# Lynne-Zheng-Linfang/HS-Pose

Hardware: AMD Instinct MI355X
Metric: point-clouds/sec (N=1028) HS-layer fwd+bwd (higher is better)
Workload: dtype f32; 1 GPU; HS stack (FaceRecon backbone -> feat) fwd+bwd, B=16/GPU N=1028 fp32, train-mode BN, random-init weights (BASELINE configs[1] shape); global_batch=16, points=1028, parallelism=dp1, hipgraph=True, split_graph=False, grad_exchange=none

## Files before the change

### hs_pose_amd/csrc/gemm_x3.hip

```cpp
#include "common.h"
#include <stdlib.h>
#include <type_traits>

namespace hsp {

using f32x16 = __attribute__((ext_vector_type(16))) float;
using bf16x8 = __attribute__((ext_vector_type(8))) __bf16;
using u32x4 = __attribute__((ext_vector_type(4))) unsigned;

struct X3Args {
    const float* A[2];
    const unsigned short* P[2];
    int lda[2], ldp[2], K[2];
    long long ps[2];
    float* C; int ldc;
    int M, N;
    const float* bias;
    const float* resid; int ldr;
    const float* cbias; int rpc;
    float alpha;
    int tiles_m, tiles_n, nsplit;
    float* ws;
    float* bn_shift;
    float* bn_part;
};

#define X3_BN 128
#define X3_BK 32

__device__ __forceinline__ void x3_split8(const float (&x)[8], u32x4& hi, u32x4& mid, u32x4& lo) {
    float r1[8], r2[8];
#pragma unroll
    for (int i = 0; i < 8; ++i) {
        const float h = __uint_as_float(__float_as_uint(x[i]) & 0xffff0000u);
        r1[i] = x[i] - h;
        const float m = __uint_as_float(__float_as_uint(r1[i]) & 0xffff0000u);
        r2[i] = r1[i] - m;
    }
#pragma unroll
    for (int i = 0; i < 4; ++i) {
        hi[i] = __builtin_amdgcn_perm(__float_as_uint(x[2 * i + 1]), __float_as_uint(x[2 * i]), 0x07060302u);
        mid[i] = __builtin_amdgcn_perm(__float_as_uint(r1[2 * i + 1]), __float_as_uint(r1[2 * i]), 0x07060302u);
        lo[i] = __builtin_amdgcn_perm(__float_as_uint(r2[2 * i + 1]), __float_as_uint(r2[2 * i]), 0x07060302u);
    }
}

template <int WM, bool TWO, int EPI, int PA = 0>
__global__ __launch_bounds__(256, 2) void gemm_x3_kernel(const X3Args g) {
    constexpr int BM = 64 * WM;
    constexpr int A_PLANE = BM * 64, B_PLANE = X3_BN * 64;
    constexpr int NAU = WM;
    extern __shared__ __attribute__((aligned(16))) char smem[];
    char* sA = smem;
    char* sB = smem + 3 * A_PLANE;

    const int tid = threadIdx.x, lane = tid & 63;
    const int wave = __builtin_amdgcn_readfirstlane(tid >> 6);
    const int li = lane & 31, lh = lane >> 5;
    const int wm0 = (wave >> 1) * 32 * WM, wn0 = (wave & 1) * 64;

    const int item = blockIdx.x;
    const int o = item / g.nsplit, ks = item - o * g.nsplit;
    const int tm = o / g.tiles_n, tn = o - tm * g.tiles_n;
    const int m0 = tm * BM, n0 = tn * X3_BN;
    const int T0 = (g.K[0] + X3_BK - 1) / X3_BK;
    const int T1 = TWO ? (g.K[1] + X3_BK - 1) / X3_BK : 0;
    const int TT = T0 + T1;
    const int per = (TT + g.nsplit - 1) / g.nsplit;
    const int t_begin = ks * per, t_end = min(TT, t_begin + per);

    f32x16 acc[WM][2];
#pragma unroll
    for (int a = 0; a < WM; ++a)
#pragma unroll
        for (int b = 0; b < 2; ++b)
#pragma unroll
            for (int r = 0; r < 16; ++r) acc[a][b][r] = 0.f;
    if constexpr (EPI == 2) {
        const __amdgpu_buffer_rsrc_t rsR = __builtin_amdgcn_make_buffer_rsrc(
            const_cast<float*>(g.resid), 0, (int)((size_t)g.M * g.ldr * 4), 0x00020000);
        const unsigned ldr4 = (unsigned)g.ldr * 4u;
#pragma unroll
        for (int y = 0; y < 2; ++y) {
            const int col = n0 + wn0 + 32 * y + li;
            const unsigned voff = col < g.N ? (unsigned)(m0 + wm0 + 4 * lh) * ldr4 + (unsigned)col * 4u : 0xfffffff0u;
#pragma unroll
            for (int x = 0; x < WM; ++x)
#pragma unroll
                for (int r = 0; r < 16; ++r)
                    acc[x][y][r] = __uint_as_float(
                        __builtin_amdgcn_raw_buffer_load_b32(rsR, voff, (unsigned)(32 * x + (r & 3) + 8 * (r >> 2)) * ldr4, 0));
        }
    }

    u32x4 bv[6];
    const __amdgpu_buffer_rsrc_t rsA0 = __builtin_amdgcn_make_buffer_rsrc(
        const_cast<float*>(g.A[0]), 0, (int)((((size_t)g.M - 1) * g.lda[0] + g.K[0]) * 4), 0x00020000);
    const __amdgpu_buffer_rsrc_t rsA1 = __builtin_amdgcn_make_buffer_rsrc(
        const_cast<float*>(TWO ? g.A[1] : g.A[0]), 0, (int)((((size_t)g.M - 1) * g.lda[TWO ? 1 : 0] + g.K[TWO ? 1 : 0]) * 4), 0x00020000);
    auto fetchA = [&](float (&dst)[NAU][8], int t) {
        const int src = (TWO && t >= T0) ? 1 : 0;
        const int kb = (src ? t - T0 : t) * X3_BK;
        const __amdgpu_buffer_rsrc_t ra = src ? rsA1 : rsA0;
        const unsigned lda = (unsigned)g.lda[src];
#pragma unroll
        for (int i = 0; i < NAU; ++i) {
            const int u = tid + 256 * i, row = u >> 2, c8 = u & 3;
            const int gr = m0 + row, k0 = kb + 8 * c8;
            const unsigned off = gr < g.M ? ((unsigned)gr * lda + (unsigned)k0) * 4u : 0xfffffff0u;
            const u32x4 v0 = __builtin_amdgcn_raw_buffer_load_b128(ra, off, 0, 0);
            const u32x4 v1 = __builtin_amdgcn_raw_buffer_load_b128(ra, off, 16, 0);
#pragma unroll
            for (int e = 0; e < 4; ++e) { dst[i][e] = __uint_as_float(v0[e]); dst[i][4 + e] = __uint_as_float(v1[e]); }
        }
    };
    auto fetchB = [&](int t) {
        const int src = (TWO && t >= T0) ? 1 : 0;
        const int kb = (src ? t - T0 : t) * X3_BK;
        const unsigned short* P = g.P[src];
        const int ldp = g.ldp[src];
        const long long ps = g.ps[src];
#pragma unroll
        for (int i = 0; i < 6; ++i) {
            const int q = tid + 256 * i, plane = q >> 9, w = q & 511, row = w >> 2, c = w & 3;
            bv[i] = *reinterpret_cast<const u32x4*>(P + plane * ps + (size_t)min(n0 + row, g.N - 1) * ldp + kb + 8 * c);
        }
    };
    auto stashA = [&](float (&srcv)[NAU][8], int t) {
        {
            const int src = (TWO && t >= T0) ? 1 : 0;
            const int kb = (src ? t - T0 : t) * X3_BK, K = g.K[src];
            if (kb + X3_BK > K) {
#pragma unroll
                for (int i = 0; i < NAU; ++i) {
                    const int k0 = kb + 8 * ((tid + 256 * i) & 3);
#pragma unroll
                    for (int e = 0; e < 8; ++e) srcv[i][e] = k0 + e < K ? srcv[i][e] : 0.f;
                }
            }
        }
#pragma unroll
        for (int i = 0; i < NAU; ++i) {
            const int u = tid + 256 * i, row = u >> 2, c8 = u & 3;
            u32x4 h, m, l;
            x3_split8(srcv[i], h, m, l);
            const int off = row * 64 + ((c8 ^ ((row >> 2) & 3)) << 4);
            *reinterpret_cast<u32x4*>(sA + off) = h;
            *reinterpret_cast<u32x4*>(sA + A_PLANE + off) = m;
            *reinterpret_cast<u32x4*>(sA + 2 * A_PLANE + off) = l;
        }
    };
    auto stashB = [&]() {
#pragma unroll
        for (int i = 0; i < 6; ++i) {
            const int q = tid + 256 * i, plane = q >> 9, w = q & 511, row = w >> 2, c = w & 3;
            *reinterpret_cast<u32x4*>(sB + plane * B_PLANE + row * 64 + ((c ^ ((row >> 2) & 3)) << 4)) = bv[i];
        }
    };
    auto mma = [&]() {
#pragma unroll
        for (int s = 0; s < 2; ++s) {
            u32x4 fa[WM][3], fb[2][3];
            const int c = 2 * s + lh;
#pragma unroll
            for (int x = 0; x < WM; ++x) {
                const int row = wm0 + 32 * x + li;
                const int off = row * 64 + ((c ^ ((row >> 2) & 3)) << 4);
#pragma unroll
                for (int p = 0; p < 3; ++p) fa[x][p] = *reinterpret_cast<const u32x4*>(sA + p * A_PLANE + off);
            }
#pragma unroll
            for (int y = 0; y < 2; ++y) {
                const int row = wn0 + 32 * y + li;
                const int off = row * 64 + ((c ^ ((row >> 2) & 3)) << 4);
#pragma unroll
                for (int p = 0; p < 3; ++p) fb[y][p] = *reinterpret_cast<const u32x4*>(sB + p * B_PLANE + off);
            }
            constexpr int SA[6] = {0, 2, 1, 0, 1, 0}, SB[6] = {2, 0, 1, 1, 0, 0};
#pragma unroll
            for (int q = 0; q < 6; ++q)
#pragma unroll
                for (int x = 0; x < WM; ++x)
#pragma unroll
                    for (int y = 0; y < 2; ++y)
                        acc[x][y] = __builtin_amdgcn_mfma_f32_32x32x16_bf16(__builtin_bit_cast(bf16x8, fa[x][SA[q]]),
                                                                            __builtin_bit_cast(bf16x8, fb[y][SB[q]]), acc[x][y], 0, 0, 0);
        }
    };
    {
        float av[NAU][8];
        if (t_begin < t_end) { fetchA(av, t_begin); fetchB(t_begin); }
        for (int t = t_begin; t < t_end; ++t) {
            __syncthreads();
            stashA(av, t);
            stashB();
            __syncthreads();
            if (t + 1 < t_end) { fetchA(av, t + 1); fetchB(t + 1); }
            mma();
        }
    }

    if (g.nsplit > 1) {
        float* wsp = g.ws + (size_t)ks * g.M * g.N;
#pragma unroll
        for (int y = 0; y < 2; ++y) {
            const int col = n0 + wn0 + 32 * y + li;
#pragma unroll
            for (int x = 0; x < WM; ++x)
#pragma unroll
                for (int r = 0; r < 16; ++r) {
                    const int row = m0 + wm0 + 32 * x + (r & 3) + 8 * (r >> 2) + 4 * lh;
                    if (row < g.M && col < g.N) wsp[(size_t)row * g.N + col] = acc[x][y][r];
                }
        }
        return;
    }
    constexpr bool HAS_BIAS = EPI & 1, HAS_RES = (EPI & 2) && EPI != 2, HAS_CB = EPI & 4, HAS_BN = EPI & 8;
    float bn1[2] = {0.f, 0.f}, bn2[2] = {0.f, 0.f};
    const int c0 = m0 / g.rpc, nb = (c0 + 1) * g.rpc;
    const bool two_clouds = g.rpc >= BM;
#pragma unroll
    for (int y = 0; y < 2; ++y) {
        const int col = n0 + wn0 + 32 * y + li;
        const bool cok = col < g.N;
        const int colc = min(col, g.N - 1);
        float bvv = 0.f, cb0 = 0.f, cb1 = 0.f, bsh = 0.f;
        if constexpr (HAS_BIAS) bvv = g.bias[colc];
        if constexpr (HAS_BN) {
            if constexpr (HAS_RES) bsh = g.resid[colc] + g.cbias[colc];
            else bsh = bvv;
            if (tm == 0 && wm0 == 0 && lh == 0 && cok) g.bn_shift[col] = bsh;
        }
        if constexpr (HAS_CB) {
            cb0 = g.cbias[(size_t)c0 * g.N + colc];
            cb1 = g.cbias[(size_t)min(c0 + 1, (g.M - 1) / g.rpc) * g.N + colc];
        }
#pragma unroll
        for (int x = 0; x < WM; ++x) {
#pragma unroll
            for (int r4 = 0; r4 < 16; r4 += 4) {
                float rv[4];
                if constexpr (HAS_RES) {
#pragma unroll
                    for (int q = 0; q < 4; ++q) {
                        const int row = min(m0 + wm0 + 32 * x + q + 8 * (r4 >> 2) + 4 * lh, g.M - 1);
                        rv[q] = g.resid[(size_t)row * g.ldr + colc];
                    }
                }
#pragma unroll
                for (int q = 0; q < 4; ++q) {
                    const int r = r4 + q;
                    const int row = m0 + wm0 + 32 * x + q + 8 * (r4 >> 2) + 4 * lh;
                    float v = g.alpha * acc[x][y][r] + bvv;
                    if constexpr (HAS_RES) v += rv[q];
                    if constexpr (HAS_CB) {
                        if (two_clouds) v += row >= nb ? cb1 : cb0;
                        else v += g.cbias[(size_t)(min(row, g.M - 1) / g.rpc) * g.N + colc];
                    }
                    if (row < g.M && cok) g.C[(size_t)row * g.ldc + col] = v;
                    if constexpr (HAS_BN) {
                        const float d = row < g.M ? v - bsh : 0.f;
                        bn1[y] += d;
                        bn2[y] += d * d;
                    }
                }
            }
        }
    }
    if constexpr (HAS_BN) {
        __syncthreads();
        float* red = reinterpret_cast<float*>(smem);
#pragma unroll
        for (int y = 0; y < 2; ++y) {
            const float a = bn1[y] + __shfl_xor(bn1[y], 32, 64), b = bn2[y] + __shfl_xor(bn2[y], 32, 64);
            if (lh == 0) {
                red[((wave >> 1) * 2 + 0) * 128 + wn0 + 32 * y + li] = a;
                red[((wave >> 1) * 2 + 1) * 128 + wn0 + 32 * y + li] = b;
            }
        }
        __syncthreads();
        if (tid < 128 && n0 + tid < g.N) {
            g.bn_part[((size_t)tm * 2 + 0) * g.N + n0 + tid] = red[0 * 128 + tid] + red[2 * 128 + tid];
            g.bn_part[((size_t)tm * 2 + 1) * g.N + n0 + tid] = red[1 * 128 + tid] + red[3 * 128 + tid];
        }
    }
}

template <int EPI>
__global__ __launch_bounds__(256, 2) void gemm_x3_panel_kernel(const X3Args g) {
    constexpr int KS = 8, K = 128, D = 2;
    constexpr int ROWB = K * 2, PLANE = 32 * ROWB, BUF = 3 * PLANE;
    constexpr int UPR = K / 8, NAU = (32 * UPR) / 256;
    extern __shared__ __attribute__((aligned(16))) char smem[];
    char* sA = smem;

    const int tid = threadIdx.x, lane = tid & 63;
    const int wave = __builtin_amdgcn_readfirstlane(tid >> 6);
    const int li = lane & 31, lh = lane >> 5;
    const int P = g.tiles_n, R = gridDim.x / P;
    const int xq = blockIdx.x / HSP_NUM_XCD, xcd = blockIdx.x % HSP_NUM_XCD;
    const int panel = xq % P, slot = (xq / P) * HSP_NUM_XCD + xcd;
    const int col = panel * 128 + 32 * wave + li;
    const int ntiles = g.tiles_m;

    const __amdgpu_buffer_rsrc_t rsA0 = __builtin_amdgcn_make_buffer_rsrc(
        const_cast<float*>(g.A[0]), 0, (int)((((size_t)g.M - 1) * g.lda[0] + g.K[0]) * 4), 0x00020000);
    auto fetchA = [&](float (&dst)[NAU][8], int tile) {
#pragma unroll
        for (int i = 0; i < NAU; ++i) {
            const int u = tid + 256 * i, row = u / UPR, k0 = 8 * (u % UPR);
            const int gr = tile * 32 + row;
            const unsigned off = gr < g.M ? ((unsigned)gr * (unsigned)g.lda[0] + (unsigned)k0) * 4u : 0xfffffff0u;
            const u32x4 v0 = __builtin_amdgcn_raw_buffer_load_b128(rsA0, off, 0, 0);
            const u32x4 v1 = __builtin_amdgcn_raw_buffer_load_b128(rsA0, off, 16, 0);
#pragma unroll
            for (int e = 0; e < 4; ++e) { dst[i][e] = __uint_as_float(v0[e]); dst[i][4 + e] = __uint_as_float(v1[e]); }
        }
    };
    auto stashA = [&](float (&srcv)[8], int unit, int buf) {
        const int u = tid + 256 * unit, row = u / UPR, c8 = u % UPR;
        u32x4 h, m, l;
        x3_split8(srcv, h, m, l);
        char* d = sA + buf * BUF + row * ROWB + ((c8 ^ (row & 15)) << 4);
        *reinterpret_cast<u32x4*>(d) = h;
        *reinterpret_cast<u32x4*>(d + PLANE) = m;
        *reinterpret_cast<u32x4*>(d + 2 * PLANE) = l;
    };

    float av[D][NAU][8];
    int t = slot;
#pragma unroll
    for (int j = 0; j < D; ++j) fetchA(av[j], t + j * R);

    u32x4 br[KS][3];
#pragma unroll
    for (int half = 0; half < 2; ++half) {
        if (half) __syncthreads();
#pragma unroll
        for (int i = 0; i < 12; ++i) {
            const int q = tid + 256 * i, p = q >> 10, n = (q >> 4) & 63, c = q & 15;
            const u32x4 v = *reinterpret_cast<const u32x4*>(g.P[0] + p * g.ps[0] + (size_t)(panel * 128 + 64 * half + n) * g.ldp[0] + 8 * c);
            *reinterpret_cast<u32x4*>(sA + (p * 64 + n) * ROWB + ((c ^ (n & 15)) << 4)) = v;
        }
        __syncthreads();
        if ((wave >> 1) == half) {
            const int n = 32 * (wave & 1) + li;
#pragma unroll
            for (int s = 0; s < KS; ++s)
#pragma unroll
                for (int p = 0; p < 3; ++p)
                    br[s][p] = *reinterpret_cast<const u32x4*>(sA + (p * 64 + n) * ROWB + (((2 * s + lh) ^ (n & 15)) << 4));
        }
    }
    float bvv = 0.f;
    if constexpr (EPI & 1) bvv = g.bias[col];
    __syncthreads();
    __builtin_amdgcn_s_waitcnt(0x0070);
    stashA(av[0][0], 0, 0);
    stashA(av[0][1], 1, 0);
    fetchA(av[0], t + D * R);
    __syncthreads();

    const __amdgpu_buffer_rsrc_t rsC = __builtin_amdgcn_make_buffer_rsrc(g.C, 0, (int)((((size_t)g.M - 1) * g.ldc + g.N) * 4), 0x00020000);
    const unsigned ldc4 = (unsigned)g.ldc * 4u;
    auto store4 = [&](const f32x16& acc, int tile, bool valid, int r0) {
        const unsigned base = valid ? (unsigned)(tile * 32 + 4 * lh) * ldc4 + (unsigned)col * 4u : 0x80000000u;
#pragma unroll
        for (int r = r0; r < r0 + 4; ++r) {
// ... 85 lines not shown
    const int tk = (Kk + 63) >> 6;
    const int n0 = (t / tk) * 32, k0 = (t % tk) * 64;
    const int lx = threadIdx.x & 31, ly = threadIdx.x >> 5;
    unsigned* dst = reinterpret_cast<unsigned*>(d.dst);
    float x0[4], x1[4];
    if (d.transpose) {
#pragma unroll
        for (int j = 0; j < 8; ++j) {
            const int k = k0 + ly + 8 * j, nn = n0 + lx;
            tile[ly + 8 * j][lx] = (k < Kk && nn < Nn) ? d.src[(size_t)k * d.ld + nn] : 0.f;
        }
        __syncthreads();
#pragma unroll
        for (int j = 0; j < 4; ++j) { x0[j] = tile[2 * lx][ly + 8 * j]; x1[j] = tile[2 * lx + 1][ly + 8 * j]; }
    } else {
#pragma unroll
        for (int j = 0; j < 4; ++j) {
            const int nn = n0 + ly + 8 * j, k = k0 + 2 * lx;
            const float* p = d.src + (size_t)min(nn, Nn - 1) * d.ld;
            x0[j] = (nn < Nn && k < Kk) ? p[k] : 0.f;
            x1[j] = (nn < Nn && k + 1 < Kk) ? p[k + 1] : 0.f;
        }
    }
#pragma unroll
    for (int j = 0; j < 4; ++j) {
        const int nn = n0 + ly + 8 * j, k = k0 + 2 * lx;
        if (nn >= Nn || k >= Kk) continue;
        float r1[2], r2[2];
        const float xs[2] = {x0[j], x1[j]};
#pragma unroll
        for (int q = 0; q < 2; ++q) {
            const float h = __uint_as_float(__float_as_uint(xs[q]) & 0xffff0000u);
            r1[q] = xs[q] - h;
            const float m = __uint_as_float(__float_as_uint(r1[q]) & 0xffff0000u);
            r2[q] = r1[q] - m;
        }
        const size_t o = ((size_t)nn * d.kp + k) >> 1;
        const size_t psd = (size_t)d.ps >> 1;
        dst[o] = __builtin_amdgcn_perm(__float_as_uint(xs[1]), __float_as_uint(xs[0]), 0x07060302u);
        dst[psd + o] = __builtin_amdgcn_perm(__float_as_uint(r1[1]), __float_as_uint(r1[0]), 0x07060302u);
        dst[2 * psd + o] = __builtin_amdgcn_perm(__float_as_uint(r2[1]), __float_as_uint(r2[0]), 0x07060302u);
    }
}

static int x3_pick_split(long long tiles, int TT) {
    constexpr int per_cu = 2;
    if (tiles >= 2 * HSP_NUM_CU || TT < 16) return 1;
    int ns = (int)((per_cu * HSP_NUM_CU + tiles - 1) / tiles);
    if (ns > TT / 8) ns = TT / 8;
    if (ns > 16) ns = 16;
    if (ns < 2) return 1;
    const int per = (TT + ns - 1) / ns;
    return (TT + per - 1) / per;
}

static int x3_pick_wm(int M, int N) {
    const long long t128 = (long long)((M + 127) / 128) * ((N + X3_BN - 1) / X3_BN);
    return t128 >= 2 * HSP_NUM_CU ? 2 : 1;
}

}

using namespace hsp;

extern "C" int hsp_split_params_x3(const HspSplitDesc* table_dev, int n, int total_tiles, hspStream_t stream) {
    if (!table_dev || n <= 0 || total_tiles <= 0) return HSP_ERR_BAD_ARG;
    hipLaunchKernelGGL(split_params_x3_kernel, dim3(total_tiles), dim3(256), 0, as_stream(stream), table_dev, n);
    return check_launch();
}

extern "C" int hsp_gemm_x3_supported(int M, int N, int K1, int K2) {
    if (!(M > 0 && N >= 64 && K1 > 0 && K2 >= 0)) return 0;
    const long long t64 = (long long)((M + 63) / 64) * ((N + X3_BN - 1) / X3_BN);
    const int TT = (K1 + X3_BK - 1) / X3_BK + (K2 > 0 ? (K2 + X3_BK - 1) / X3_BK : 0);
    return (t64 >= 128 || TT >= 32) ? 1 : 0;
}

extern "C" size_t hsp_gemm_x3_workspace_bytes(int M, int N, int K1, int K2) {
    if (!hsp_gemm_x3_supported(M, N, K1, K2)) return 0;
    const int wm = x3_pick_wm(M, N), bm = 64 * wm;
    const int TT = (K1 + X3_BK - 1) / X3_BK + (K2 > 0 ? (K2 + X3_BK - 1) / X3_BK : 0);
    const int ns = x3_pick_split((long long)((M + bm - 1) / bm) * ((N + X3_BN - 1) / X3_BN), TT);
    return ns > 1 ? (size_t)ns * M * N * sizeof(float) : 0;
}

static int gemm_x3_impl(const float* A1, int lda1, const hsp_bf16_t* P1, int ldp1, long long ps1, int K1,
                        const float* A2, int lda2, const hsp_bf16_t* P2, int ldp2, long long ps2, int K2, int M, int N,
                        const float* bias, const float* resid, int ldr, const float* cloud_bias, int rows_per_cloud,
                        float alpha, float* C, int ldc, void* ws, size_t ws_bytes, float* bn_shift, float* bn_part,
                        hspStream_t stream) {
    if (!A1 || !P1 || !C || M <= 0 || N <= 0 || K1 <= 0 || lda1 < K1 || ldc < N) return HSP_ERR_BAD_ARG;
    const bool two = A2 != nullptr;
    if (two && (!P2 || K2 <= 0 || lda2 < K2)) return HSP_ERR_BAD_ARG;
    if (!two) K2 = 0;
    if (resid && ldr < N) return HSP_ERR_BAD_ARG;
    if (cloud_bias && rows_per_cloud <= 0) return HSP_ERR_BAD_ARG;
    if (!hsp_gemm_x3_supported(M, N, K1, K2)) return HSP_ERR_UNSUPPORTED;
    if ((long long)M * lda1 * 4 >= (1ll << 31) || (two && (long long)M * lda2 * 4 >= (1ll << 31))) return HSP_ERR_UNSUPPORTED;
    auto al16 = [](const void* q, long long ld, int es) { return ((reinterpret_cast<size_t>(q) | ((size_t)ld * es)) & 15) == 0; };
    const int kp1 = (K1 + X3_BK - 1) / X3_BK * X3_BK, kp2 = (K2 + X3_BK - 1) / X3_BK * X3_BK;
    if (!al16(A1, lda1, 4) || !al16(P1, ldp1, 2) || (ps1 & 7) || ldp1 < kp1) return HSP_ERR_UNSUPPORTED;
    if (two && (!al16(A2, lda2, 4) || !al16(P2, ldp2, 2) || (ps2 & 7) || ldp2 < kp2)) return HSP_ERR_UNSUPPORTED;
    X3Args g{};
    g.A[0] = A1; g.P[0] = P1; g.lda[0] = lda1; g.ldp[0] = ldp1; g.K[0] = K1; g.ps[0] = ps1;
    g.A[1] = A2; g.P[1] = P2; g.lda[1] = lda2; g.ldp[1] = ldp2; g.K[1] = K2; g.ps[1] = ps2;
    g.C = C; g.ldc = ldc; g.M = M; g.N = N; g.bias = bias; g.resid = resid; g.ldr = ldr;
    g.cbias = cloud_bias; g.rpc = rows_per_cloud > 0 ? rows_per_cloud : 1; g.alpha = alpha;
    g.bn_shift = bn_shift; g.bn_part = bn_part;
    const bool bn = bn_shift != nullptr;
    const bool bn_out = bn && resid && cloud_bias && !bias, bn_lin = bn && bias && !resid && !cloud_bias && !two;
    if (bn && (!bn_part || !(bn_out || bn_lin))) return HSP_ERR_UNSUPPORTED;
    hipStream_t st = as_stream(stream);
    {
        const int epi0 = (bias ? 1 : 0) | (resid ? 2 : 0) | (cloud_bias ? 4 : 0);
        if (!bn && !two && epi0 <= 1 && K1 == 128 && N % 128 == 0 && (long long)(M + 32) * ldc * 4 < (1ll << 31)) {
            const int P = N / 128;
            const int R = (2 * HSP_NUM_CU / P) / HSP_NUM_XCD * HSP_NUM_XCD;
            const int nt = (M + 31) / 32;
            const int rounds = R ? (nt + R - 1) / R : 0;
            if (R && rounds >= 3 && (double)nt / ((double)rounds * R) >= 0.75) {
                g.tiles_m = nt; g.tiles_n = P; g.nsplit = 1; g.ws = nullptr;
                const dim3 pgrid((unsigned)(P * R)), pblock(256);
                const size_t lds = (size_t)2 * 3 * 32 * 128 * 2;
#define X3_PANEL(EPI_)                                                                                                    \
    do {                                                                                                                  \
        auto kern = gemm_x3_panel_kernel<EPI_>;                                                                           \
        static bool attr_set = false;                                                                                     \
        if (!attr_set) {                                                                                                  \
            hipError_t e = hipFuncSetAttribute(reinterpret_cast<const void*>(kern), hipFuncAttributeMaxDynamicSharedMemorySize, (int)lds); \
            if (e != hipSuccess) { set_last_hip_error(e); return HSP_ERR_LAUNCH; }                                        \
            attr_set = true;                                                                                              \
        }                                                                                                                 \
        hipLaunchKernelGGL(kern, pgrid, pblock, lds, st, g);                                                              \
    } while (0)
                if (epi0) X3_PANEL(1);
                else X3_PANEL(0);
#undef X3_PANEL
                return check_launch();
            }
        }
    }
    const int wm = bn_out ? 1 : x3_pick_wm(M, N), bm = 64 * wm;
    g.tiles_m = (M + bm - 1) / bm; g.tiles_n = (N + X3_BN - 1) / X3_BN;
    const int TT = (K1 + X3_BK - 1) / X3_BK + (two ? (K2 + X3_BK - 1) / X3_BK : 0);
    const int epi = (bias ? 1 : 0) | (resid ? 2 : 0) | (cloud_bias ? 4 : 0);
    int ns = epi ? 1 : x3_pick_split((long long)g.tiles_m * g.tiles_n, TT);
    if (ns > 1 && (!ws || (size_t)ns * M * N * sizeof(float) > ws_bytes)) ns = 1;
    g.nsplit = ns; g.ws = ns > 1 ? reinterpret_cast<float*>(ws) : nullptr;
    const long long items = (long long)g.tiles_m * g.tiles_n * ns;
    if (items > (1ll << 30)) return HSP_ERR_UNSUPPORTED;
    const dim3 grid((unsigned)items), block(256);
    if (epi != 0 && epi != 1 && epi != 6 && !(epi == 2 && !two && alpha == 1.0f) && !(epi == 4 && !two)) return HSP_ERR_UNSUPPORTED;
    if (bn_out) {
        if (two) hipLaunchKernelGGL((gemm_x3_kernel<1, true, 14, 0>), grid, block, 3 * (size_t)(64 + X3_BN) * 64, st, g);
        else hipLaunchKernelGGL((gemm_x3_kernel<1, false, 14, 0>), grid, block, 3 * (size_t)(64 + X3_BN) * 64, st, g);
        return check_launch();
    }
    if (bn_lin) {
        if (g.tiles_m > 512) return HSP_ERR_UNSUPPORTED;
        if (wm == 2) hipLaunchKernelGGL((gemm_x3_kernel<2, false, 9, 0>), grid, block, 3 * (size_t)(128 + X3_BN) * 64, st, g);
        else hipLaunchKernelGGL((gemm_x3_kernel<1, false, 9, 0>), grid, block, 3 * (size_t)(64 + X3_BN) * 64, st, g);
        return check_launch();
    }
#define X3_K(WM_, TWO_, EPI_, PA_)                                                                                 \
    do {                                                                                                           \
        auto kern = gemm_x3_kernel<WM_, TWO_, EPI_, PA_>;                                                          \
        const size_t lds = 3 * (size_t)(64 * WM_ + X3_BN) * 64;                                                    \
        hipLaunchKernelGGL(kern, grid, block, lds, st, g);                                                         \
    } while (0)
#define X3_LAUNCH(WM_, PA_)                                        \
    do {                                                           \
        if (two) {                                                 \
            if (epi == 0) X3_K(WM_, true, 0, PA_);                 \
            else if (epi == 1) X3_K(WM_, true, 1, PA_);            \
            else X3_K(WM_, true, 6, PA_);                          \
        } else {                                                   \
            if (epi == 0) X3_K(WM_, false, 0, PA_);                \
            else if (epi == 1) X3_K(WM_, false, 1, PA_);           \
            else if (epi == 2) X3_K(WM_, false, 2, 0);             \
            else if (epi == 4) X3_K(WM_, false, 4, 0);             \
            else X3_K(WM_, false, 6, PA_);                         \
        }                                                          \
    } while (0)
    if (wm == 2) X3_LAUNCH(2, 0);
    else X3_LAUNCH(1, 0);
#undef X3_LAUNCH
#undef X3_K
    int rc = check_launch();
    if (rc || ns == 1) return rc;
    const long long total = (long long)M * N;
    long long rg = (total / 4 + 255) / 256;
    if (rg > HSP_NUM_CU * 8) rg = HSP_NUM_CU * 8;
    hipLaunchKernelGGL(gemm_x3_reduce_kernel, dim3((unsigned)rg), dim3(256), 0, st, g.ws, ns, total, N, alpha, C, ldc);
    return check_launch();
}

extern "C" int hsp_gemm_x3_bn_tiles(int M, int N) {
    if (M <= 0 || N <= 0) return 0;
    return (M + 64 * x3_pick_wm(M, N) - 1) / (64 * x3_pick_wm(M, N));
}
extern "C" int hsp_gemm_x3_bias_bn_f32(const float* A1, int lda1, const hsp_bf16_t* P1, int ldp1, long long ps1, int K1, int M, int N,
                                       const float* bias, float* C, int ldc, float* bn_shift, float* bn_part, hspStream_t stream) {
    if (!bn_shift || !bn_part || !bias) return HSP_ERR_BAD_ARG;
    return gemm_x3_impl(A1, lda1, P1, ldp1, ps1, K1, nullptr, 0, nullptr, 0, 0, 0, M, N, bias, nullptr, 0, nullptr, 0, 1.0f, C, ldc,
                        nullptr, 0, bn_shift, bn_part, stream);
}

namespace hsp {

#define SR_MAXM 16

__global__ __launch_bounds__(256) void small_rows_nt_kernel(const float* __restrict__ A, int lda, const float* __restrict__ W, int ldw,
                                                            int M, int N, int K, float alpha, float* __restrict__ out, int ldo) {
    extern __shared__ float sA[];
    for (int e = threadIdx.x; e < M * K; e += 256) sA[e] = A[(size_t)(e / K) * lda + (e % K)];
    __syncthreads();
    const int lane = threadIdx.x & 63, wave = threadIdx.x >> 6;
    for (int n = blockIdx.x * 8 + wave; n < min(N, (int)blockIdx.x * 8 + 8); n += 4) {
        float p[SR_MAXM];
#pragma unroll
        for (int m = 0; m < SR_MAXM; ++m) p[m] = 0.f;
        for (int k = lane; k < K; k += 64) {
            const float w = W[(size_t)n * ldw + k];
#pragma unroll
            for (int m = 0; m < SR_MAXM; ++m)
                if (m < M) p[m] = __fmaf_rn(sA[m * K + k], w, p[m]);
        }
#pragma unroll
        for (int m = 0; m < SR_MAXM; ++m) {
#pragma unroll
            for (int o = 32; o >= 1; o >>= 1) p[m] += __shfl_xor(p[m], o, 64);
        }
        if (lane == 0) {
#pragma unroll
            for (int m = 0; m < SR_MAXM; ++m)
// ... 190 lines not shown
```

### hs_pose_amd/parallel.py

```python
import os
from typing import Iterable, List

import torch
import torch.distributed as dist


def init_distributed():
    world = int(os.environ.get("WORLD_SIZE", "1"))
    force = os.environ.get("HSP_FORCE_DIST", "0") == "1"
    rank = int(os.environ.get("RANK", "0"))
    local = int(os.environ.get("LOCAL_RANK", "0"))
    use_cuda = torch.cuda.is_available()
    device = torch.device(os.environ.get("HSP_DIST_DEVICE") or f"cuda:{local}") if use_cuda else torch.device("cpu")
    if use_cuda:
        torch.cuda.set_device(device)
    backend = os.environ.get("HSP_DIST_BACKEND") or ("nccl" if use_cuda else "gloo")
    if (world > 1 or force) and not dist.is_initialized():
        os.environ.setdefault("MASTER_ADDR", "127.0.0.1")
        os.environ.setdefault("MASTER_PORT", "29500")
        os.environ.setdefault("HSA_ENABLE_IPC_MODE_LEGACY", "0")
        if backend == "nccl":
            dist.init_process_group("nccl", rank=rank, world_size=world, device_id=device)
        else:
            dist.init_process_group(backend, rank=rank, world_size=world)
# ... 69 lines not shown
    def _on_grad(self, p):
        bi = self._bucket_of[p]
        self._pending[bi] -= 1
        if self._pending[bi] == 0:
            self._launch(bi)

    def _launch(self, bi):
        flat, off = self._flat[bi], 0
        for p in self.buckets[bi]:
            n = p.numel()
            g = p.grad if p.grad is not None else torch.zeros_like(p)
            flat[off:off + n].copy_(g.reshape(-1))
            off += n
        self._works[bi] = all_reduce_(flat, group=self.group, async_op=True)

    def finish(self):
        if self.world == 1:
            return
        for bi in range(len(self.buckets)):
            if self._works[bi] is None:
                self._launch(bi)
        inv = 1.0 / self.world
        for bi, b in enumerate(self.buckets):
            self._works[bi].wait()
            flat, off = self._flat[bi], 0
            flat.mul_(inv)
            for p in b:
                n = p.numel()
                if p.grad is None:
                    p.grad = flat[off:off + n].view_as(p).clone()
                else:
                    p.grad.copy_(flat[off:off + n].view_as(p))
                off += n
            self._works[bi] = None
        self._pending = [len(b) for b in self.buckets]

    def close(self):
        for h in self._handles:
            h.remove()
        self._handles = []


def graphed_step_with_exchange(graphed, world, group=None):
    if not getattr(graphed, "split", False):
        graphed.run()
        if world > 1 or dist.is_initialized():
            all_reduce_(graphed.flat_grad, group=group)
            graphed.flat_grad.mul_(1.0 / world)
        return
    graphed.run_first()
    late = all_reduce_(graphed.flat_late, group=group, async_op=True)
    graphed.run_second()
    early = all_reduce_(graphed.flat_early, group=group, async_op=True)
    late.wait()
    early.wait()
    graphed.flat_grad.mul_(1.0 / world)


def mean_flat_gradients(buffers, group=None):
    if not dist.is_initialized():
        return
    world = dist.get_world_size(group)
    if world == 1:
        return
    works = [all_reduce_(b, group=group, async_op=True) for b in buffers]
    for w in works:
        w.wait()
    inv = 1.0 / world
    for b in buffers:
        b.mul_(inv)


def choose_exchange_form(forms, world, group=None, replays=3, sync=None, forced=None, probe_single_rank=False):
    import time
    names = [n for n in ("split", "single") if forms.get(n) is not None]
    if not names:
        return None, {"reason": "no captured form"}
    if forced in names:
        return forced, {"reason": f"forced by HSP_SPLIT_GRAPH ({forced})"}
    if len(names) == 1 or (world == 1 and not probe_single_rank) or not dist.is_initialized():
        pick = names[0] if world > 1 or len(names) == 1 else "single"
        return pick, {"reason": "only one form captured" if len(names) == 1 else "one rank: nothing to overlap"}
    sync = sync or (lambda: None)
    times = {}
    for n in names:
        graphed_step_with_exchange(forms[n], world, group)
        sync(); dist.barrier(group)
        t0 = time.perf_counter()
        for _ in range(replays):
            graphed_step_with_exchange(forms[n], world, group)
        sync()
        t = torch.tensor([time.perf_counter() - t0], dtype=torch.float64)
        dist.barrier(group)
        gathered = [None] * dist.get_world_size(group)
        dist.all_gather_object(gathered, float(t.item()), group=group)
        times[n] = 1e3 * max(gathered) / replays
    decision = ["split" if times["split"] <= 1.03 * times["single"] else "single"]
    dist.broadcast_object_list(decision, src=0, group=group)
    return decision[0], {"reason": "start-up probe (max over ranks, rank 0 decides; split kept unless single is > 3 % faster)",
                         "probe_ms_per_step": {k: round(v, 4) for k, v in times.items()}, "replays": replays}
```

Baseline: 9125 point-clouds/sec.

## Add persistent multi-stage ring GEMM kernel with direct global-to-LDS loads

Adds a persistent gemm_x3 ring kernel that streams A and packed B tiles straight into LDS through global_load_lds, using an S-stage ring buffer (2 or 4 deep) so loads overlap the MFMA work. Each block loops over several work items. The accumulator init and epilogue are factored into shared helpers. The ring path is chosen by default when N<=256, there is no K-split, and K is a multiple of the tile. A is now staged as raw fp32 in LDS, so the hi/mid/lo split presumably happens in the mma step, which can move work and change register pressure and occupancy. The multi-rank exchange probe is also changed to alternate forms and compare the fastest step, which does not matter on one rank.

```diff
diff --git a/hs_pose_amd/csrc/gemm_x3.hip b/hs_pose_amd/csrc/gemm_x3.hip
--- a/hs_pose_amd/csrc/gemm_x3.hip
+++ b/hs_pose_amd/csrc/gemm_x3.hip
@@ -45,37 +45,20 @@
     }
 }
 
-template <int WM, bool TWO, int EPI, int PA = 0>
-__global__ __launch_bounds__(256, 2) void gemm_x3_kernel(const X3Args g) {
+template <int WM, int EPI>
+__device__ __forceinline__ void x3_acc_init(const X3Args& g, f32x16 (&acc)[WM][2], int tm, int tn, int tid) {
+#pragma unroll
+    for (int a = 0; a < WM; ++a)
+#pragma unroll
+        for (int b = 0; b < 2; ++b)
+#pragma unroll
+            for (int r = 0; r < 16; ++r) acc[a][b][r] = 0.f;
     constexpr int BM = 64 * WM;
-    constexpr int A_PLANE = BM * 64, B_PLANE = X3_BN * 64;
-    constexpr int NAU = WM;
-    extern __shared__ __attribute__((aligned(16))) char smem[];
-    char* sA = smem;
-    char* sB = smem + 3 * A_PLANE;
-
-    const int tid = threadIdx.x, lane = tid & 63;
+    const int lane = tid & 63;
     const int wave = __builtin_amdgcn_readfirstlane(tid >> 6);
     const int li = lane & 31, lh = lane >> 5;
     const int wm0 = (wave >> 1) * 32 * WM, wn0 = (wave & 1) * 64;
-
-    const int item = blockIdx.x;
-    const int o = item / g.nsplit, ks = item - o * g.nsplit;
-    const int tm = o / g.tiles_n, tn = o - tm * g.tiles_n;
     const int m0 = tm * BM, n0 = tn * X3_BN;
-    const int T0 = (g.K[0] + X3_BK - 1) / X3_BK;
-    const int T1 = TWO ? (g.K[1] + X3_BK - 1) / X3_BK : 0;
-    const int TT = T0 + T1;
-    const int per = (TT + g.nsplit - 1) / g.nsplit;
-    const int t_begin = ks * per, t_end = min(TT, t_begin + per);
-
-    f32x16 acc[WM][2];
-#pragma unroll
-    for (int a = 0; a < WM; ++a)
-#pragma unroll
-        for (int b = 0; b < 2; ++b)
-#pragma unroll
-            for (int r = 0; r < 16; ++r) acc[a][b][r] = 0.f;
     if constexpr (EPI == 2) {
         const __amdgpu_buffer_rsrc_t rsR = __builtin_amdgcn_make_buffer_rsrc(
             const_cast<float*>(g.resid), 0, (int)((size_t)g.M * g.ldr * 4), 0x00020000);
@@ -92,114 +75,16 @@
                         __builtin_amdgcn_raw_buffer_load_b32(rsR, voff, (unsigned)(32 * x + (r & 3) + 8 * (r >> 2)) * ldr4, 0));
         }
     }
-
-    u32x4 bv[6];
-    const __amdgpu_buffer_rsrc_t rsA0 = __builtin_amdgcn_make_buffer_rsrc(
-        const_cast<float*>(g.A[0]), 0, (int)((((size_t)g.M - 1) * g.lda[0] + g.K[0]) * 4), 0x00020000);
-    const __amdgpu_buffer_rsrc_t rsA1 = __builtin_amdgcn_make_buffer_rsrc(
-        const_cast<float*>(TWO ? g.A[1] : g.A[0]), 0, (int)((((size_t)g.M - 1) * g.lda[TWO ? 1 : 0] + g.K[TWO ? 1 : 0]) * 4), 0x00020000);
-    auto fetchA = [&](float (&dst)[NAU][8], int t) {
-        const int src = (TWO && t >= T0) ? 1 : 0;
-        const int kb = (src ? t - T0 : t) * X3_BK;
-        const __amdgpu_buffer_rsrc_t ra = src ? rsA1 : rsA0;
-        const unsigned lda = (unsigned)g.lda[src];
-#pragma unroll
-        for (int i = 0; i < NAU; ++i) {
-            const int u = tid + 256 * i, row = u >> 2, c8 = u & 3;
-            const int gr = m0 + row, k0 = kb + 8 * c8;
-            const unsigned off = gr < g.M ? ((unsigned)gr * lda + (unsigned)k0) * 4u : 0xfffffff0u;
-            const u32x4 v0 = __builtin_amdgcn_raw_buffer_load_b128(ra, off, 0, 0);
-            const u32x4 v1 = __builtin_amdgcn_raw_buffer_load_b128(ra, off, 16, 0);
-#pragma unroll
-            for (int e = 0; e < 4; ++e) { dst[i][e] = __uint_as_float(v0[e]); dst[i][4 + e] = __uint_as_float(v1[e]); }
-        }
-    };
-    auto fetchB = [&](int t) {
-        const int src = (TWO && t >= T0) ? 1 : 0;
-        const int kb = (src ? t - T0 : t) * X3_BK;
-        const unsigned short* P = g.P[src];
-        const int ldp = g.ldp[src];
-        const long long ps = g.ps[src];
-#pragma unroll
-        for (int i = 0; i < 6; ++i) {
-            const int q = tid + 256 * i, plane = q >> 9, w = q & 511, row = w >> 2, c = w & 3;
-            bv[i] = *reinterpret_cast<const u32x4*>(P + plane * ps + (size_t)min(n0 + row, g.N - 1) * ldp + kb + 8 * c);
-        }
-    };
-    auto stashA = [&](float (&srcv)[NAU][8], int t) {
-        {
-            const int src = (TWO && t >= T0) ? 1 : 0;
-            const int kb = (src ? t - T0 : t) * X3_BK, K = g.K[src];
-            if (kb + X3_BK > K) {
-#pragma unroll
-                for (int i = 0; i < NAU; ++i) {
-                    const int k0 = kb + 8 * ((tid + 256 * i) & 3);
-#pragma unroll
-                    for (int e = 0; e < 8; ++e) srcv[i][e] = k0 + e < K ? srcv[i][e] : 0.f;
-                }
-            }
-        }
-#pragma unroll
-        for (int i = 0; i < NAU; ++i) {
-            const int u = tid + 256 * i, row = u >> 2, c8 = u & 3;
-            u32x4 h, m, l;
-            x3_split8(srcv[i], h, m, l);
-            const int off = row * 64 + ((c8 ^ ((row >> 2) & 3)) << 4);
-            *reinterpret_cast<u32x4*>(sA + off) = h;
-            *reinterpret_cast<u32x4*>(sA + A_PLANE + off) = m;
-            *reinterpret_cast<u32x4*>(sA + 2 * A_PLANE + off) = l;
-        }
-    };
-    auto stashB = [&]() {
-#pragma unroll
-        for (int i = 0; i < 6; ++i) {
-            const int q = tid + 256 * i, plane = q >> 9, w = q & 511, row = w >> 2, c = w & 3;
-            *reinterpret_cast<u32x4*>(sB + plane * B_PLANE + row * 64 + ((c ^ ((row >> 2) & 3)) << 4)) = bv[i];
-        }
-    };
-    auto mma = [&]() {
-#pragma unroll
-        for (int s = 0; s < 2; ++s) {
-            u32x4 fa[WM][3], fb[2][3];
-            const int c = 2 * s + lh;
-#pragma unroll
-            for (int x = 0; x < WM; ++x) {
-                const int row = wm0 + 32 * x + li;
-                const int off = row * 64 + ((c ^ ((row >> 2) & 3)) << 4);
-#pragma unroll
-                for (int p = 0; p < 3; ++p) fa[x][p] = *reinterpret_cast<const u32x4*>(sA + p * A_PLANE + off);
-            }
-#pragma unroll
-            for (int y = 0; y < 2; ++y) {
-                const int row = wn0 + 32 * y + li;
-                const int off = row * 64 + ((c ^ ((row >> 2) & 3)) << 4);
-#pragma unroll
-                for (int p = 0; p < 3; ++p) fb[y][p] = *reinterpret_cast<const u32x4*>(sB + p * B_PLANE + off);
-            }
-            constexpr int SA[6] = {0, 2, 1, 0, 1, 0}, SB[6] = {2, 0, 1, 1, 0, 0};
-#pragma unroll
-            for (int q = 0; q < 6; ++q)
-#pragma unroll
-                for (int x = 0; x < WM; ++x)
-#pragma unroll
-                    for (int y = 0; y < 2; ++y)
-                        acc[x][y] = __builtin_amdgcn_mfma_f32_32x32x16_bf16(__builtin_bit_cast(bf16x8, fa[x][SA[q]]),
-                                                                            __builtin_bit_cast(bf16x8, fb[y][SB[q]]), acc[x][y], 0, 0, 0);
-        }
-    };
-    {
-        float av[NAU][8];
-        if (t_begin < t_end) { fetchA(av, t_begin); fetchB(t_begin); }
-        for (int t = t_begin; t < t_end; ++t) {
-            __syncthreads();
-            stashA(av, t);
-            stashB();
-            __syncthreads();
-            if (t + 1 < t_end) { fetchA(av, t + 1); fetchB(t + 1); }
-            mma();
-        }
-    }
-
+}
+
+template <int WM, int EPI>
+__device__ __forceinline__ void x3_epilogue(const X3Args& g, f32x16 (&acc)[WM][2], int tm, int tn, int ks, int tid, char* red_area) {
+    constexpr int BM = 64 * WM;
+    const int lane = tid & 63;
+    const int wave = __builtin_amdgcn_readfirstlane(tid >> 6);
+    const int li = lane & 31, lh = lane >> 5;
+    const int wm0 = (wave >> 1) * 32 * WM, wn0 = (wave & 1) * 64;
+    const int m0 = tm * BM, n0 = tn * X3_BN;
     if (g.nsplit > 1) {
         float* wsp = g.ws + (size_t)ks * g.M * g.N;
 #pragma unroll
@@ -269,7 +154,7 @@
     }
     if constexpr (HAS_BN) {
         __syncthreads();
-        float* red = reinterpret_cast<float*>(smem);
+        float* red = reinterpret_cast<float*>(red_area);
 #pragma unroll
         for (int y = 0; y < 2; ++y) {
             const float a = bn1[y] + __shfl_xor(bn1[y], 32, 64), b = bn2[y] + __shfl_xor(bn2[y], 32, 64);
@@ -284,6 +169,268 @@
             g.bn_part[((size_t)tm * 2 + 1) * g.N + n0 + tid] = red[1 * 128 + tid] + red[3 * 128 + tid];
         }
     }
+}
+
+template <int WM, bool TWO, int EPI, int PA = 0>
+__global__ __launch_bounds__(256, 2) void gemm_x3_kernel(const X3Args g) {
+    constexpr int BM = 64 * WM;
+    constexpr int A_PLANE = BM * 64, B_PLANE = X3_BN * 64;
+    constexpr int NAU = WM;
+    extern __shared__ __attribute__((aligned(16))) char smem[];
+    char* sA = smem;
+    char* sB = smem + 3 * A_PLANE;
+
+    const int tid = threadIdx.x, lane = tid & 63;
+    const int wave = __builtin_amdgcn_readfirstlane(tid >> 6);
+    const int li = lane & 31, lh = lane >> 5;
+    const int wm0 = (wave >> 1) * 32 * WM, wn0 = (wave & 1) * 64;
+
+    const int item = blockIdx.x;
+    const int o = item / g.nsplit, ks = item - o * g.nsplit;
+    const int tm = o / g.tiles_n, tn = o - tm * g.tiles_n;
+    const int m0 = tm * BM, n0 = tn * X3_BN;
+    const int T0 = (g.K[0] + X3_BK - 1) / X3_BK;
+    const int T1 = TWO ? (g.K[1] + X3_BK - 1) / X3_BK : 0;
+    const int TT = T0 + T1;
+    const int per = (TT + g.nsplit - 1) / g.nsplit;
+    const int t_begin = ks * per, t_end = min(TT, t_begin + per);
+
+    f32x16 acc[WM][2];
+    x3_acc_init<WM, EPI>(g, acc, tm, tn, tid);
+
+    u32x4 bv[6];
+    const __amdgpu_buffer_rsrc_t rsA0 = __builtin_amdgcn_make_buffer_rsrc(
+        const_cast<float*>(g.A[0]), 0, (int)((((size_t)g.M - 1) * g.lda[0] + g.K[0]) * 4), 0x00020000);
+    const __amdgpu_buffer_rsrc_t rsA1 = __builtin_amdgcn_make_buffer_rsrc(
+        const_cast<float*>(TWO ? g.A[1] : g.A[0]), 0, (int)((((size_t)g.M - 1) * g.lda[TWO ? 1 : 0] + g.K[TWO ? 1 : 0]) * 4), 0x00020000);
+    auto fetchA = [&](float (&dst)[NAU][8], int t) {
+        const int src = (TWO && t >= T0) ? 1 : 0;
+        const int kb = (src ? t - T0 : t) * X3_BK;
+        const __amdgpu_buffer_rsrc_t ra = src ? rsA1 : rsA0;
+        const unsigned lda = (unsigned)g.lda[src];
+#pragma unroll
+        for (int i = 0; i < NAU; ++i) {
+            const int u = tid + 256 * i, row = u >> 2, c8 = u & 3;
+            const int gr = m0 + row, k0 = kb + 8 * c8;
+            const unsigned off = gr < g.M ? ((unsigned)gr * lda + (unsigned)k0) * 4u : 0xfffffff0u;
+            const u32x4 v0 = __builtin_amdgcn_raw_buffer_load_b128(ra, off, 0, 0);
+            const u32x4 v1 = __builtin_amdgcn_raw_buffer_load_b128(ra, off, 16, 0);
+#pragma unroll
+            for (int e = 0; e < 4; ++e) { dst[i][e] = __uint_as_float(v0[e]); dst[i][4 + e] = __uint_as_float(v1[e]); }
+        }
+    };
+    auto fetchB = [&](int t) {
+        const int src = (TWO && t >= T0) ? 1 : 0;
+        const int kb = (src ? t - T0 : t) * X3_BK;
+        const unsigned short* P = g.P[src];
+        const int ldp = g.ldp[src];
+        const long long ps = g.ps[src];
+#pragma unroll
+        for (int i = 0; i < 6; ++i) {
+            const int q = tid + 256 * i, plane = q >> 9, w = q & 511, row = w >> 2, c = w & 3;
+            bv[i] = *reinterpret_cast<const u32x4*>(P + plane * ps + (size_t)min(n0 + row, g.N - 1) * ldp + kb + 8 * c);
+        }
+    };
+    auto stashA = [&](float (&srcv)[NAU][8], int t) {
+        {
+            const int src = (TWO && t >= T0) ? 1 : 0;
+            const int kb = (src ? t - T0 : t) * X3_BK, K = g.K[src];
+            if (kb + X3_BK > K) {
+#pragma unroll
+                for (int i = 0; i < NAU; ++i) {
+                    const int k0 = kb + 8 * ((tid + 256 * i) & 3);
+#pragma unroll
+                    for (int e = 0; e < 8; ++e) srcv[i][e] = k0 + e < K ? srcv[i][e] : 0.f;
+                }
+            }
+        }
+#pragma unroll
+        for (int i = 0; i < NAU; ++i) {
+            const int u = tid + 256 * i, row = u >> 2, c8 = u & 3;
+            u32x4 h, m, l;
+            x3_split8(srcv[i], h, m, l);
+            const int off = row * 64 + ((c8 ^ ((row >> 2) & 3)) << 4);
+            *reinterpret_cast<u32x4*>(sA + off) = h;
+            *reinterpret_cast<u32x4*>(sA + A_PLANE + off) = m;
+            *reinterpret_cast<u32x4*>(sA + 2 * A_PLANE + off) = l;
+        }
+    };
+    auto stashB = [&]() {
+#pragma unroll
+        for (int i = 0; i < 6; ++i) {
+            const int q = tid + 256 * i, plane = q >> 9, w = q & 511, row = w >> 2, c = w & 3;
+            *reinterpret_cast<u32x4*>(sB + plane * B_PLANE + row * 64 + ((c ^ ((row >> 2) & 3)) << 4)) = bv[i];
+        }
+    };
+    auto mma = [&]() {
+#pragma unroll
+        for (int s = 0; s < 2; ++s) {
+            u32x4 fa[WM][3], fb[2][3];
+            const int c = 2 * s + lh;
+#pragma unroll
+            for (int x = 0; x < WM; ++x) {
+                const int row = wm0 + 32 * x + li;
+                const int off = row * 64 + ((c ^ ((row >> 2) & 3)) << 4);
+#pragma unroll
+                for (int p = 0; p < 3; ++p) fa[x][p] = *reinterpret_cast<const u32x4*>(sA + p * A_PLANE + off);
+            }
+#pragma unroll
+            for (int y = 0; y < 2; ++y) {
+                const int row = wn0 + 32 * y + li;
+                const int off = row * 64 + ((c ^ ((row >> 2) & 3)) << 4);
+#pragma unroll
+                for (int p = 0; p < 3; ++p) fb[y][p] = *reinterpret_cast<const u32x4*>(sB + p * B_PLANE + off);
+            }
+            constexpr int SA[6] = {0, 2, 1, 0, 1, 0}, SB[6] = {2, 0, 1, 1, 0, 0};
+#pragma unroll
+            for (int q = 0; q < 6; ++q)
+#pragma unroll
+                for (int x = 0; x < WM; ++x)
+#pragma unroll
+                    for (int y = 0; y < 2; ++y)
+                        acc[x][y] = __builtin_amdgcn_mfma_f32_32x32x16_bf16(__builtin_bit_cast(bf16x8, fa[x][SA[q]]),
+                                                                            __builtin_bit_cast(bf16x8, fb[y][SB[q]]), acc[x][y], 0, 0, 0);
+        }
+    };
+    {
+        float av[NAU][8];
+        if (t_begin < t_end) { fetchA(av, t_begin); fetchB(t_begin); }
+        for (int t = t_begin; t < t_end; ++t) {
+            __syncthreads();
+            stashA(av, t);
+            stashB();
+            __syncthreads();
+            if (t + 1 < t_end) { fetchA(av, t + 1); fetchB(t + 1); }
+            mma();
+        }
+    }
+
+    x3_epilogue<WM, EPI>(g, acc, tm, tn, ks, tid, smem);
+}
+
+#define X3R_P (X3_BN * 64)
+#define X3R_RED 2048
+
+template <int WM>
+constexpr int x3r_a() { return 64 * WM * 128; }
+template <int WM>
+constexpr int x3r_stage() { return x3r_a<WM>() + 3 * X3R_P; }
+constexpr bool x3_ring_wm2_ok(int epi) { return epi == 0 || epi == 1 || epi == 2 || epi == 9; }
+template <int S, int WM, int EPI>
+constexpr size_t x3_ring_lds() { return (size_t)S * x3r_stage<WM>() + ((EPI & 8) ? X3R_RED : 0); }
+
+__device__ __forceinline__ void x3_glds16(const void* src, char* lds_base) {
+    __builtin_amdgcn_global_load_lds((const __attribute__((address_space(1))) void*)src,
+                                     (__attribute__((address_space(3))) void*)lds_base, 16, 0, 0);
+}
+
+template <int S, int WM, bool TWO, int EPI>
+__global__ __launch_bounds__(256, S == 2 ? 2 : 1) void gemm_x3_ring_kernel(const X3Args g) {
+    static_assert(S >= 2 && S <= 4, "ring depth");
+    constexpr int X3R_A = x3r_a<WM>(), X3R_STAGE = x3r_stage<WM>();
+    constexpr int VMW = (2 * WM + 6) * (S - 2);
+    constexpr unsigned WAIT = (VMW & 15) | ((VMW >> 4) << 14) | 0x0070u | 0x0f00u;
+    extern __shared__ __attribute__((aligned(16))) char smem[];
+    char* red_area = smem + S * X3R_STAGE;
+
+    const int tid = threadIdx.x, lane = tid & 63;
+    const int wave = __builtin_amdgcn_readfirstlane(tid >> 6);
+    const int li = lane & 31, lh = lane >> 5;
+    const int wm0 = (wave >> 1) * 32 * WM, wn0 = (wave & 1) * 64;
+    const int T0 = g.K[0] / X3_BK, T1 = TWO ? g.K[1] / X3_BK : 0, TT = T0 + T1;
+    const int per = (TT + g.nsplit - 1) / g.nsplit;
+    const int n_items = g.tiles_m * g.tiles_n * g.nsplit;
+    const int G = gridDim.x;
+
+    int l_item = blockIdx.x, l_t = 0, l_te = 0, l_m0 = 0, l_n0 = 0, l_slot = 0;
+    auto l_seek = [&]() {
+        const int it = min(l_item, n_items - 1);
+        const int o = it / g.nsplit, ks = it - o * g.nsplit;
+        const int tm = o / g.tiles_n, tn = o - tm * g.tiles_n;
+        l_m0 = tm * 64 * WM; l_n0 = tn * X3_BN;
+        l_t = ks * per; l_te = min(TT, l_t + per);
+    };
+    const int a_row0 = tid >> 3, a_c0 = (tid & 7) ^ ((a_row0 >> 1) & 7);
+    auto issue = [&]() {
+        const int src = (TWO && l_t >= T0) ? 1 : 0;
+        const int kb = (src ? l_t - T0 : l_t) * X3_BK;
+        const float* A = g.A[src];
+        const unsigned short* P = g.P[src];
+        const int lda = g.lda[src], ldp = g.ldp[src];
+        const long long ps = g.ps[src];
+        char* sa = smem + l_slot * X3R_STAGE;
+        char* sb = sa + X3R_A;
+#pragma unroll
+        for (int i = 0; i < 2 * WM; ++i) {
+            const int row = min(l_m0 + a_row0 + 32 * i, g.M - 1);
+            x3_glds16(A + (size_t)row * lda + kb + 4 * a_c0, sa + (256 * i + 64 * wave) * 16);
+        }
+#pragma unroll
+        for (int i = 0; i < 6; ++i) {
+            const int q = tid + 256 * i, plane = q >> 9, w = q & 511, row = w >> 2, c = (w & 3) ^ ((row >> 2) & 3);
+            x3_glds16(P + plane * ps + (size_t)min(l_n0 + row, g.N - 1) * ldp + kb + 8 * c, sb + (256 * i + 64 * wave) * 16);
+        }
+        l_slot = l_slot + 1 == S ? 0 : l_slot + 1;
+        if (++l_t == l_te) { l_item += G; l_seek(); }
+    };
+    auto mma = [&](f32x16 (&acc)[WM][2], const char* sa, const char* sb) {
+#pragma unroll
+        for (int s = 0; s < 2; ++s) {
+            const int c0 = 4 * s + 2 * lh;
+            u32x4 fa[WM][3], fb[2][3];
+#pragma unroll
+            for (int x = 0; x < WM; ++x) {
+                const int arow = wm0 + 32 * x + li, akey = (arow >> 1) & 7;
+                const u32x4 x0 = *reinterpret_cast<const u32x4*>(sa + arow * 128 + ((c0 ^ akey) << 4));
+                const u32x4 x1 = *reinterpret_cast<const u32x4*>(sa + arow * 128 + (((c0 + 1) ^ akey) << 4));
+                float xv[8];
+#pragma unroll
+                for (int e = 0; e < 4; ++e) { xv[e] = __uint_as_float(x0[e]); xv[4 + e] = __uint_as_float(x1[e]); }
+                x3_split8(xv, fa[x][0], fa[x][1], fa[x][2]);
+            }
+            const int c = 2 * s + lh;
+#pragma unroll
+            for (int y = 0; y < 2; ++y) {
+                const int row = wn0 + 32 * y + li;
+                const int off = row * 64 + ((c ^ ((row >> 2) & 3)) << 4);
+#pragma unroll
+                for (int p = 0; p < 3; ++p) fb[y][p] = *reinterpret_cast<const u32x4*>(sb + p * X3R_P + off);
+            }
+            constexpr int SA[6] = {0, 2, 1, 0, 1, 0}, SB[6] = {2, 0, 1, 1, 0, 0};
+#pragma unroll
+            for (int q = 0; q < 6; ++q)
+#pragma unroll
+                for (int x = 0; x < WM; ++x)
+#pragma unroll
+                    for (int y = 0; y < 2; ++y)
+                        acc[x][y] = __builtin_amdgcn_mfma_f32_32x32x16_bf16(__builtin_bit_cast(bf16x8, fa[x][SA[q]]),
+                                                                            __builtin_bit_cast(bf16x8, fb[y][SB[q]]), acc[x][y], 0, 0, 0);
+        }
+    };
+
+    l_seek();
+#pragma unroll
+    for (int p = 0; p < S - 1; ++p) issue();
+    int c_slot = 0;
+    for (int item = blockIdx.x; item < n_items; item += G) {
+        const int o = item / g.nsplit, ks = item - o * g.nsplit;
+        const int tm = o / g.tiles_n, tn = o - tm * g.tiles_n;
+        const int t_begin = ks * per, t_end = min(TT, t_begin + per);
+        f32x16 acc[WM][2];
+        x3_acc_init<WM, EPI>(g, acc, tm, tn, tid);
+        for (int t = t_begin; t < t_end; ++t) {
+            __builtin_amdgcn_s_waitcnt(WAIT);
+            asm volatile("" ::: "memory");
+            __builtin_amdgcn_s_barrier();
+            asm volatile("" ::: "memory");
+            issue();
+            const char* sa = smem + c_slot * X3R_STAGE;
+            mma(acc, sa, sa + X3R_A);
+            c_slot = c_slot + 1 == S ? 0 : c_slot + 1;
+        }
+        x3_epilogue<WM, EPI>(g, acc, tm, tn, ks, tid, red_area);
+    }
+    __builtin_amdgcn_s_waitcnt(0x0f70u);
 }
 
 template <int EPI>
@@ -535,6 +682,23 @@
     const int TT = (K1 + X3_BK - 1) / X3_BK + (K2 > 0 ? (K2 + X3_BK - 1) / X3_BK : 0);
     const int ns = x3_pick_split((long long)((M + bm - 1) / bm) * ((N + X3_BN - 1) / X3_BN), TT);
     return ns > 1 ? (size_t)ns * M * N * sizeof(float) : 0;
+}
+
+static int x3_ring_mode() {
+    static const int m = [] { const char* e = getenv("HSP_X3_RING"); return e ? atoi(e) : -1; }();
+    return m;
+}
+static int x3_ring_depth() {
+    static const int d = [] { const char* e = getenv("HSP_X3_RING_S"); const int v = e ? atoi(e) : 2; return v == 4 ? 4 : 2; }();
+    return x3_ring_mode() == 0 ? 0 : d;
+}
+static int x3_ring_wm() {
+    static const int w = [] { const char* e = getenv("HSP_X3_RING_WM"); return e && atoi(e) == 2 ? 2 : 1; }();
+    return w;
+}
+static bool x3_ring_wanted(int M, int N, int TT, int ns, int epi, bool bn) {
+    if (x3_ring_mode() == 1) return true;
+    return N <= 256 && ns == 1;
 }
 
 static int gemm_x3_impl(const float* A1, int lda1, const hsp_bf16_t* P1, int ldp1, long long ps1, int K1,
@@ -604,6 +768,57 @@
     if (items > (1ll << 30)) return HSP_ERR_UNSUPPORTED;
     const dim3 grid((unsigned)items), block(256);
     if (epi != 0 && epi != 1 && epi != 6 && !(epi == 2 && !two && alpha == 1.0f) && !(epi == 4 && !two)) return HSP_ERR_UNSUPPORTED;
+    {
+        const int S = x3_ring_depth();
+        const int rwm = bn_lin ? wm : (bn_out || !x3_ring_wm2_ok(epi)) ? 1 : x3_ring_wm();
+        if (S && K1 % X3_BK == 0 && K2 % X3_BK == 0 && x3_ring_wanted(M, N, TT, ns, epi, bn)) {
+            g.tiles_m = (M + 64 * rwm - 1) / (64 * rwm);
+            const long long ritems = (long long)g.tiles_m * g.tiles_n * ns;
+            const dim3 rgrid((unsigned)persistent_blocks(ritems, S == 2 ? 2 : 1));
+            const int repi = bn ? (bn_out ? 14 : 9) : epi;
+#define X3_RK(S_, TWO_, EPI_)                                                                                             \
+    do {                                                                                                                  \
+        constexpr int W2_ = x3_ring_wm2_ok(EPI_) ? 2 : 1;                                                                 \
+        auto kern = rwm == 2 ? gemm_x3_ring_kernel<S_, W2_, TWO_, EPI_> : gemm_x3_ring_kernel<S_, 1, TWO_, EPI_>;          \
+        const size_t lds = rwm == 2 ? x3_ring_lds<S_, W2_, EPI_>() : x3_ring_lds<S_, 1, EPI_>();                          \
+        static bool attr_set[2] = {false, false};                                                                         \
+        if (!attr_set[rwm - 1]) {                                                                                         \
+            hipError_t e = hipFuncSetAttribute(reinterpret_cast<const void*>(kern), hipFuncAttributeMaxDynamicSharedMemorySize, (int)lds); \
+            if (e != hipSuccess) { set_last_hip_error(e); return HSP_ERR_LAUNCH; }                                        \
+            attr_set[rwm - 1] = true;                                                                                     \
+        }                                                                                                                 \
+        hipLaunchKernelGGL(kern, rgrid, block, lds, st, g);                                                               \
+    } while (0)
+#define X3_RL(S_)                                                  \
+    do {                                                           \
+        if (two) {                                                 \
+            if (repi == 0) X3_RK(S_, true, 0);                     \
+            else if (repi == 1) X3_RK(S_, true, 1);                \
+            else if (repi == 14) X3_RK(S_, true, 14);              \
+            else X3_RK(S_, true, 6);                               \
+        } else {                                                   \
+            if (repi == 0) X3_RK(S_, false, 0);                    \
+            else if (repi == 1) X3_RK(S_, false, 1);               \
+            else if (repi == 2) X3_RK(S_, false, 2);               \
+            else if (repi == 4) X3_RK(S_, false, 4);               \
+            else if (repi == 9) X3_RK(S_, false, 9);               \
+            else if (repi == 14) X3_RK(S_, false, 14);             \
+            else X3_RK(S_, false, 6);                              \
+        }                                                          \
+    } while (0)
+            if (S == 2) X3_RL(2);
+            else X3_RL(4);
+#undef X3_RL
+#undef X3_RK
+            int rc = check_launch();
+            if (rc || ns == 1) return rc;
+            const long long total = (long long)M * N;
+            long long rg = (total / 4 + 255) / 256;
+            if (rg > HSP_NUM_CU * 8) rg = HSP_NUM_CU * 8;
+            hipLaunchKernelGGL(gemm_x3_reduce_kernel, dim3((unsigned)rg), dim3(256), 0, st, g.ws, ns, total, N, alpha, C, ldc);
+            return check_launch();
+        }
+    }
     if (bn_out) {
         if (two) hipLaunchKernelGGL((gemm_x3_kernel<1, true, 14, 0>), grid, block, 3 * (size_t)(64 + X3_BN) * 64, st, g);
         else hipLaunchKernelGGL((gemm_x3_kernel<1, false, 14, 0>), grid, block, 3 * (size_t)(64 + X3_BN) * 64, st, g);
diff --git a/hs_pose_amd/parallel.py b/hs_pose_amd/parallel.py
--- a/hs_pose_amd/parallel.py
+++ b/hs_pose_amd/parallel.py
@@ -175,20 +175,27 @@
         pick = names[0] if world > 1 or len(names) == 1 else "single"
         return pick, {"reason": "only one form captured" if len(names) == 1 else "one rank: nothing to overlap"}
     sync = sync or (lambda: None)
-    times = {}
     for n in names:
         graphed_step_with_exchange(forms[n], world, group)
-        sync(); dist.barrier(group)
-        t0 = time.perf_counter()
-        for _ in range(replays):
+    sync(); dist.barrier(group)
+    steps = {n: [] for n in names}
+    t0 = time.perf_counter()
+    for _ in range(replays):
+        for n in names:
             graphed_step_with_exchange(forms[n], world, group)
-        sync()
-        t = torch.tensor([time.perf_counter() - t0], dtype=torch.float64)
-        dist.barrier(group)
-        gathered = [None] * dist.get_world_size(group)
-        dist.all_gather_object(gathered, float(t.item()), group=group)
-        times[n] = 1e3 * max(gathered) / replays
-    decision = ["split" if times["split"] <= 1.03 * times["single"] else "single"]
+            sync()
+            t1 = time.perf_counter()
+            steps[n].append(t1 - t0)
+            t0 = t1
+    dist.barrier(group)
+    gathered = [None] * dist.get_world_size(group)
+    dist.all_gather_object(gathered, steps, group=group)
+    per_step = {n: [1e3 * max(g[n][i] for g in gathered) for i in range(replays)] for n in names}
+    times = {n: sum(v) / replays for n, v in per_step.items()}
+    best = {n: min(v) for n, v in per_step.items()}
+    decision = ["split" if best["split"] <= 1.03 * best["single"] else "single"]
     dist.broadcast_object_list(decision, src=0, group=group)
-    return decision[0], {"reason": "start-up probe (max over ranks, rank 0 decides; split kept unless single is > 3 % faster)",
-                         "probe_ms_per_step": {k: round(v, 4) for k, v in times.items()}, "replays": replays}
+    return decision[0], {"reason": "start-up probe (forms alternated, max over ranks per step, fastest step; rank 0 decides; split "
+                                   "kept unless single is > 3 % faster)",
+                         "probe_ms_per_step": {k: round(v, 4) for k, v in times.items()},
+                         "probe_best_ms": {k: round(v, 4) for k, v in best.items()}, "replays": replays}
```

Result: no change. 9146 point-clouds/sec, median of 5 (+0.2%).
